# muyangyi/SimSeg

Measured on AMD Instinct MI355X. Metric: image-text pairs/sec (train) + seg images/sec (eval), ViT-B, higher is better.
Workload: dtype fp16

## Files before the change

### include/simseg_hip.h

```cpp
#ifndef SIMSEG_HIP_H
#define SIMSEG_HIP_H
#include <stdint.h>
#ifdef __cplusplus
extern "C" {
#endif

int simseg_version(void);
int simseg_set_half_type(int t);
const char* simseg_last_error(void);

int simseg_gemm(const void* A, const void* B, void* C, int64_t M, int64_t N, int64_t K, int64_t lda, int64_t ldb,
                int64_t ldc, int in_dtype, int out_dtype, int transA, int transB, float alpha, const float* bias,
                const float* rowscale, const float* residual, int64_t ldr, int act, const void* aux, void* aux_out,
                int row_group, int res_mod, int accumulate, int splitk, uint64_t drop_seed, float drop_p, float* colsum,
                void* stream);
int simseg_gemm_aux_blocked_ok(int64_t M, int64_t N, int64_t K);

int simseg_patch_text_sim(const void* x, const void* text, float* out, int64_t M, int64_t C, int64_t K, int dtype, float eps,
                          int normalize, void* stream);

int simseg_set_gemm_variant(int v);
int simseg_gemm_last_variant(void);

int simseg_layernorm_fwd(const float* x, const float* gamma, const float* beta, void* y, int out_dtype, void* y_bf16,
                         float* mean, float* rstd, int64_t rows, int64_t D, float eps, void* stream);
int simseg_layernorm_bwd(const void* dy_bf16, const float* dy_f32, const float* dres, const void* dres_bf16, const float* x,
                         const void* y_bf16, const float* beta, const float* mean,
                         const float* rstd, const float* gamma, float* dx_f32, void* dx_bf16, float* dgamma,
                         float* dbeta, float* dxsum, float* partials, int64_t rows, int64_t D, uint64_t drop_seed, float drop_p,
                         void* stream);
int64_t simseg_layernorm_bwd_workspace_bytes(int64_t rows, int64_t D);

int simseg_colsum_accum(const void* in, int in_dtype, float* out, int64_t rows, int64_t N, int64_t ld, void* stream);

int simseg_vit_im2col(const float* image, void* cols, int out_dtype, int64_t B, int64_t H, int64_t W, void* stream);
int simseg_vit_cls_rows(const float* cls, const float* pos, float* x, int64_t B, int64_t T, int64_t D, void* stream);
int simseg_vit_cls_grad(const float* dx, float* dcls, int64_t B, int64_t T, int64_t D, void* stream);

int simseg_bert_embed_fwd(const int64_t* ids, const float* word, const float* pos, const float* type0, float* out,
                          int64_t B, int64_t L, int64_t D, int64_t vocab, void* stream);
int simseg_bert_embed_bwd(const int64_t* ids, const int64_t* mask, const float* dsum, float* dword, int64_t B, int64_t L,
                          int64_t D, int64_t vocab, void* stream);

int simseg_topk_pool_l2norm_fwd(const void* tok, int dtype, const int64_t* mask, float* emb, int32_t* idx, float* norm,
                                float* scratch, int64_t B, int64_t N, int64_t P, int k, float eps, int normalize, void* stream);
int64_t simseg_topk_pool_workspace_bytes(int64_t B, int64_t P, int k);
int simseg_topk_pool_l2norm_bwd(const float* demb, const float* emb, const float* norm, const int32_t* idx, void* dtok,
                                int dtype, int64_t B, int64_t N, int64_t P, int k, float eps, int normalize, void* stream);

int simseg_set_attention_variant(int v);
int simseg_debug_attn_trace(void* buf);
int simseg_debug_gemm_trace(void* buf);
int simseg_debug_gemm_stagger(int ticks);
int simseg_debug_gemm_wgrad_blocks(int blocks);

// ... 143 lines not shown
```

### simseg_amd/csrc/gemm.hip

```cpp
#include "common.h"

#ifdef SS_GEMM_ABLATE
#define SS_ABL(v) (p.stagger == (v))
#else
#define SS_ABL(v) false
#endif

namespace {

constexpr int BM = 128, BN = 128, NTHREADS = 256;
constexpr int MC_PITCH = 320;
template <int KB> struct Geo {
    static constexpr int KC_PITCH = KB + 16;
    static constexpr int NCH = KB / 16;
    static constexpr int LOADS = 128 * NCH / NTHREADS;
    static constexpr int KROWS = KB / 2;
    static constexpr int TILE_BYTES = (128 * KC_PITCH > KROWS * MC_PITCH) ? 128 * KC_PITCH : KROWS * MC_PITCH;
    static constexpr int KSTEPS = KB / 32;
};

struct GemmParams {
    const void* A; const void* B; void* C;
    int M, N, K;
    long lda, ldb, ldc;
    float alpha;
    const float* bias;
    const float* rowscale;
    const float* residual;
    long ldr;
    int act;
    const void* aux;
    void* aux_out;
    int row_group;
// ... 988 lines not shown
    const int cl = lane & 31, h2 = lane >> 5;
    const float bL = p.bias ? p.bias[c0 + cl] : 0.f, bR = p.bias ? p.bias[c1 + cl] : 0.f;
    float* Cf = reinterpret_cast<float*>(p.C);
    f32x16 rl[2], rr[2];
    auto load_res = [&](int i, f32x16& xl, f32x16& xr) {
        const int row0 = m0 + (i >> 1) * 128 + grp * 64 + (i & 1) * 32;
#pragma unroll
        for (int e = 0; e < 16; ++e) {
            const long ro = (long)(row0 + (e & 3) + 8 * (e >> 2) + 4 * h2) * p.ldr;
            xl[e] = __builtin_nontemporal_load(p.residual + ro + c0 + cl);
            xr[e] = __builtin_nontemporal_load(p.residual + ro + c1 + cl);
        }
    };
    if (p.residual) load_res(0, rl[0], rr[0]);
#pragma unroll
    for (int i = 0; i < 4; ++i) {
        if (p.residual && i < 3) load_res(i + 1, rl[(i + 1) & 1], rr[(i + 1) & 1]);
        const int row0 = m0 + (i >> 1) * 128 + grp * 64 + (i & 1) * 32;
#pragma unroll
        for (int e = 0; e < 16; ++e) {
            const int row = row0 + (e & 3) + 8 * (e >> 2) + 4 * h2;
            float vl = acc[i][0][e] * p.alpha + bL, vr = acc[i][1][e] * p.alpha + bR;
            if (p.drop_thresh) {
                vl = dropout_keep(p.drop_seed, (unsigned long long)row * p.N + c0 + cl, p.drop_thresh) ? vl * p.drop_scale : 0.f;
                vr = dropout_keep(p.drop_seed, (unsigned long long)row * p.N + c1 + cl, p.drop_thresh) ? vr * p.drop_scale : 0.f;
            }
            if (p.residual) { vl += rl[i & 1][e]; vr += rr[i & 1][e]; }
            Cf[(long)row * p.ldc + c0 + cl] = vl;
            Cf[(long)row * p.ldc + c1 + cl] = vr;
        }
    }
}

template <typename TO, bool TA, bool TB, int PP_LEAD = 4, int PRIO = 1, int BIG = 0, int EK = 1>
__global__ __launch_bounds__(512, 2) void gemm_pp_kernel(GemmParams p) {
    extern __shared__ __attribute__((aligned(16))) char lds[];
    const int tid = threadIdx.x, lane = tid & 63, wave = __builtin_amdgcn_readfirstlane(tid >> 6);
    const int grp = wave >> 2, wn = wave & 3;
    const int tiles_n = (p.N + 255) / 256;
    const int tiles = tiles_n * ((p.M + 255) / 256);
    const int q = xcd_remap(blockIdx.x, gridDim.x);
    const int kz = q / tiles, t = q - kz * tiles;
    const int m0 = (t / tiles_n) * 256, n0 = (t % tiles_n) * 256;
    const int nk = p.K / 64;
    const int kt0 = kz * p.ksplit;
    const int ntile = min(nk, kt0 + p.ksplit) - kt0;
    const int stot = 4 * ntile;
    const char* Ab = static_cast<const char*>(p.A) + (TA ? (long)kt0 * 64 * p.lda * 2 : (long)kt0 * 128);
    const char* Bb = static_cast<const char*>(p.B) + (TB ? (long)kt0 * 64 * p.ldb * 2 : (long)kt0 * 128);
    const long astep = TA ? 64 * p.lda * 2 : 128, bstep = TB ? 64 * p.ldb * 2 : 128;
    long dA = 0, dB = 0;
    bool pf_ok = false;
    if (BIG && p.pf_next && p.nsplit == 1) {
        const int nb8 = (int)gridDim.x >> 3, rr8 = (int)gridDim.x & 7, xx = (int)blockIdx.x & 7, jj = (int)blockIdx.x >> 3;
        if (jj + 32 < nb8 + (xx < rr8 ? 1 : 0)) {
            const int tn_ = t + 32;
            const int m1 = (tn_ / tiles_n) * 256, n1 = (tn_ % tiles_n) * 256;
            if (m0 + 256 <= p.M && n0 + 256 <= p.N && m1 + 256 <= p.M && n1 + 256 <= p.N) {
                pf_ok = true;
                dA = TA ? (long)(m1 - m0) * 2 : (long)(m1 - m0) * p.lda * 2;
                dB = TB ? (long)(n1 - n0) * 2 : (long)(n1 - n0) * p.ldb * 2;
            }
        }
    }
    unsigned offA[2][2], offB[2][2];
#pragma unroll
    for (int h = 0; h < 2; ++h)
#pragma unroll
        for (int i = 0; i < 2; ++i) {
            offA[h][i] = pp_src_off<TA>(wave * 2 + i, lane, m0 + h * 128, p.M, p.lda);
            offB[h][i] = pp_src_off<TB>(wave * 2 + i, lane, n0 + h * 128, p.N, p.ldb);
            asm volatile("" : "+v"(offA[h][i]), "+v"(offB[h][i]));
        }
    const unsigned lds0 = (unsigned)(unsigned long)(__attribute__((address_space(3))) char*)lds;
    PPFrag<TA, 2> fra;
// ... 112 lines not shown
#undef PP_CLUSTER
    if (!pf_ok) wait_vm<0>();
    if (grp == 0) __builtin_amdgcn_s_barrier();
    if (p.dbg_trace) tr2 = wall_clock64();

    const bool atomic = p.nsplit > 1;
    const bool vec_ok = epilogue_vec_ok(p, sizeof(TO));
    float* wlds = reinterpret_cast<float*>(lds) + wave * EP_WAVE_FLOATS;
    float cs[8] = {0.f, 0.f, 0.f, 0.f, 0.f, 0.f, 0.f, 0.f};
    const int c0 = n0 + wn * 32, c1 = c0 + 128;
    if constexpr (sizeof(TO) == 2) {
        const bool fastep = !atomic && vec_ok && !p.residual && !p.rowscale && p.row_group == 0 && !p.drop_thresh && !p.dbg_skip_epilogue &&
                            (p.act == 0 || p.act == 1 || (p.act == 3 && (!p.aux_blocked || (EK == 2 && p.aux_blocked == 1) || (EK == 4 && p.aux_blocked == 2))) ||
                             (((EK == 1 && !p.aux_blocked) || (EK == 3 && p.aux_blocked == 1) || (EK == 5 && p.aux_blocked == 2)) && p.act == 4 && p.aux)) && (p.act == 4 || !p.colsum) &&
                            m0 + 256 <= p.M && n0 + 256 <= p.N;
        if (fastep) {
            pp_epilogue_bf16<EK>(p, acc, reinterpret_cast<char*>(wlds), m0, c0, c1, grp, lane);
            if (pf_ok) wait_vm<16>();
            if (p.dbg_trace && tid == 0) {
                const unsigned long long tr3 = wall_clock64();
                asm volatile("s_waitcnt vmcnt(0)" ::: "memory");
                unsigned long long* d = p.dbg_trace + (long)blockIdx.x * 5;
                d[0] = tr0; d[1] = tr1; d[2] = tr2; d[3] = wall_clock64(); d[4] = tr3;
            }
            return;
        }
    }
    if constexpr (sizeof(TO) == 4) {
        const bool direct = !atomic && !p.rowscale && !p.aux && p.act == 0 && p.row_group == 0 && !p.colsum && !p.accumulate &&
                            !p.dbg_skip_epilogue && m0 + 256 <= p.M && n0 + 256 <= p.N;
        if (direct) {
            pp_epilogue_f32_direct(p, acc, m0, c0, c1, grp, lane);
            if (pf_ok) wait_vm<63>();
            if (p.dbg_trace && tid == 0) {
                const unsigned long long tr3 = wall_clock64();
                asm volatile("s_waitcnt vmcnt(0)" ::: "memory");
                unsigned long long* d = p.dbg_trace + (long)blockIdx.x * 5;
                d[0] = tr0; d[1] = tr1; d[2] = tr2; d[3] = wall_clock64(); d[4] = tr3;
            }
            return;
        }
    }
#pragma unroll 1
    for (int i = 0; i < 4; ++i) {
        f32x16 l = acc[0][0], r = acc[0][1];
#pragma unroll
        for (int ii = 1; ii < 4; ++ii)
            if (ii == i) { l = acc[ii][0]; r = acc[ii][1]; }
        if (p.dbg_trace && tid == 0) p.dbg_trace[(long)gridDim.x * 5 + (long)blockIdx.x * 4 + i] = wall_clock64();
        epilogue_block<TO>(p, l, r, wlds, m0 + (i >> 1) * 128 + grp * 64 + (i & 1) * 32, c0, c1, lane, atomic, vec_ok, cs);
    }
    flush_colsum(p, cs, c0, c1, lane);
    if (pf_ok) wait_vm<0>();
    if (p.dbg_trace && tid == 0) {
        const unsigned long long tr3 = wall_clock64();
        asm volatile("s_waitcnt vmcnt(0)" ::: "memory");
        unsigned long long* d = p.dbg_trace + (long)blockIdx.x * 5;
        d[0] = tr0; d[1] = tr1; d[2] = tr2; d[3] = wall_clock64(); d[4] = tr3;
    }
}

template <typename TO, bool TA, bool TB, int LEAD = 4, int PRIO = 1, int BIG = 0, int EK = 1>
int launch_pp(const GemmParams& p, int splitk, hipStream_t stream) {
    constexpr int SMEM = 9 * PP_HALF;
    static bool configured = false;
    auto kern = gemm_pp_kernel<TO, TA, TB, LEAD, PRIO, BIG, EK>;
// ... 485 lines not shown
    return 0;
}
extern "C" int simseg_debug_gemm_trace(void* buf) { g_gemm_debug_trace = static_cast<unsigned long long*>(buf); return 0; }

extern "C" int simseg_set_gemm_variant(int v) {
#ifndef SS_HALF
    simseg_set_gemm_variant_h16(v);
#endif
    g_gemm_debug_skip_epilogue = v >= 100;
    g_gemm_variant = v % 100;
    return 0;
}

namespace {
}

extern "C" int simseg_patch_text_sim(const void* x, const void* text, float* out, int64_t M, int64_t C, int64_t K, int dtype,
                                     float eps, int normalize, void* stream) {
    SS_HALF_FWD(simseg_patch_text_sim, x, text, out, M, C, K, dtype, eps, normalize, stream);
    SS_CHECK(x && text && out, "patch_text_sim: null pointer");
    SS_CHECK(M > 0 && C > 0 && C <= 256 && K > 0 && M < (1ll << 31), "patch_text_sim: need 1 <= C <= 256 (got C=%lld)", (long long)C);
    SS_CHECK(dtype == 0 || dtype == 1, "patch_text_sim: dtype must be 0 (fp32) or 1 (bf16)");
    const int epc = dtype == 0 ? 4 : 8;
    SS_CHECK(K % epc == 0 && ((uintptr_t)x % 16) == 0 && ((uintptr_t)text % 16) == 0, "patch_text_sim: K must be a multiple of %d and the operands 16-byte aligned", epc);
    if (dtype == 0) return dispatch_simmap<float>(x, text, out, (int)M, (int)C, (int)K, eps, normalize, (hipStream_t)stream);
    return dispatch_simmap<bf16_t>(x, text, out, (int)M, (int)C, (int)K, eps, normalize, (hipStream_t)stream);
}

extern "C" int simseg_gemm_aux_blocked_ok(int64_t M, int64_t N, int64_t K) {
    if (M <= 0 || N <= 0 || K <= 0 || M % 256 || N % 256 || K % 64 || K < 768) return 0;
    return (M / 256) * (N / 256) >= 96;
}

extern "C" int simseg_gemm(const void* A, const void* B, void* C, int64_t M, int64_t N, int64_t K, int64_t lda,
                           int64_t ldb, int64_t ldc, int in_dtype, int out_dtype, int transA, int transB, float alpha,
                           const float* bias, const float* rowscale, const float* residual, int64_t ldr, int act,
                           const void* aux, void* aux_out, int row_group, int res_mod, int accumulate, int splitk,
                           uint64_t drop_seed, float drop_p, float* colsum, void* stream) {
    SS_HALF_FWD(simseg_gemm, A, B, C, M, N, K, lda, ldb, ldc, in_dtype, out_dtype, transA, transB, alpha, bias, rowscale, residual, ldr, act, aux, aux_out, row_group, res_mod, accumulate, splitk, drop_seed, drop_p, colsum, stream);
    SS_CHECK(A && B && C, "simseg_gemm: null operand");
    SS_CHECK(M > 0 && N > 0 && K > 0 && M < (1ll << 31) && N < (1ll << 31) && K < (1ll << 31), "simseg_gemm: bad shape %lld x %lld x %lld",
             (long long)M, (long long)N, (long long)K);
    const int epc = in_dtype == 0 ? 4 : 8;
    SS_CHECK(in_dtype == 0 || in_dtype == 1, "simseg_gemm: in_dtype must be 0 (fp32) or 1 (bf16)");
    SS_CHECK(out_dtype == 0 || out_dtype == 1, "simseg_gemm: out_dtype must be 0 (fp32) or 1 (bf16)");
    SS_CHECK(in_dtype == 1 || out_dtype == 0, "simseg_gemm: fp32 operands produce fp32 output");
    SS_CHECK(in_dtype == 1 || (!transA && !transB), "simseg_gemm: transposed operands need bf16");
    SS_CHECK(!(transA && !transB), "simseg_gemm: (transA, !transB) is not on the path");
    const bool aligned = ((uintptr_t)A % 16) == 0 && ((uintptr_t)B % 16) == 0 && lda % epc == 0 && ldb % epc == 0 &&
                         (transA ? M : K) % epc == 0 && (transB ? N : K) % epc == 0;
    SS_CHECK(aligned || in_dtype == 0, "simseg_gemm: bf16 operands need 16-byte aligned pointers and contiguous extents / leading dimensions that are multiples of 8");
    SS_CHECK(((uintptr_t)A % 4) == 0 && ((uintptr_t)B % 4) == 0, "simseg_gemm: misaligned operand");
    SS_CHECK(splitk <= 1 || (out_dtype == 0 && act == 0 && !bias && !residual && drop_p == 0.f && !colsum),
             "simseg_gemm: split-K needs a plain fp32 accumulate epilogue");
    SS_CHECK(drop_p >= 0.f && drop_p < 1.f, "simseg_gemm: dropout p out of range");
    SS_CHECK(act >= 0 && act <= 8, "simseg_gemm: act must be 0..8");
    const int blocked = act >= 7 ? 2 : (act >= 5 ? 1 : 0);
    if (blocked) {
        const bool fwd = act == 5 || act == 7;
        SS_CHECK(simseg_gemm_aux_blocked_ok(M, N, K) && in_dtype == 1 && out_dtype == 1 && !transA && !rowscale && !residual && row_group == 0 &&
                 drop_p == 0.f && splitk <= 1 && ldc == N && (fwd ? aux_out != nullptr : aux != nullptr) &&
                 ((uintptr_t)(fwd ? aux_out : aux) % 16) == 0 && ((uintptr_t)C % 16) == 0 && (!bias || ((uintptr_t)bias % 16) == 0),
                 "simseg_gemm: act %d needs a full-tile 16-bit problem on the ping-pong kernel (simseg_gemm_aux_blocked_ok) with a plain epilogue", act);
        act = fwd ? 3 : 4;
    }
    SS_CHECK((act != 2 && act != 4) || aux, "simseg_gemm: act=2/4 needs aux");
// ... 29 lines not shown
```

### simseg_amd/csrc/half_names.h

```cpp
#pragma once
#ifdef SS_HALF
#define simseg_gemm_last_variant simseg_gemm_last_variant_h16
#define simseg_debug_gemm_stagger simseg_debug_gemm_stagger_h16
#define simseg_debug_gemm_wgrad_blocks simseg_debug_gemm_wgrad_blocks_h16
#define simseg_debug_gemm_trace simseg_debug_gemm_trace_h16
#define simseg_set_gemm_variant simseg_set_gemm_variant_h16
#define simseg_patch_text_sim simseg_patch_text_sim_h16
#define simseg_gemm_aux_blocked_ok simseg_gemm_aux_blocked_ok_h16
#define simseg_gemm simseg_gemm_h16
#define simseg_colsum_accum simseg_colsum_accum_h16
#define simseg_debug_attn_trace simseg_debug_attn_trace_h16
#define simseg_set_attention_variant simseg_set_attention_variant_h16
#define simseg_attention_fwd simseg_attention_fwd_h16
#define simseg_attention_fwd_qscaled simseg_attention_fwd_qscaled_h16
#define simseg_attention_fwd_x3 simseg_attention_fwd_x3_h16
#define simseg_debug_attention_timeline simseg_debug_attention_timeline_h16
#define simseg_attention_bwd_workspace_bytes simseg_attention_bwd_workspace_bytes_h16
#define simseg_attention_bwd simseg_attention_bwd_h16
#define simseg_attention_fwd_rows simseg_attention_fwd_rows_h16
#define simseg_attention_bwd_rows simseg_attention_bwd_rows_h16
#define simseg_attention_fwd_planes simseg_attention_fwd_planes_h16
#define simseg_attention_bwd_planes simseg_attention_bwd_planes_h16
#define simseg_layernorm_fwd simseg_layernorm_fwd_h16
#define simseg_layernorm_bwd simseg_layernorm_bwd_h16
#define simseg_layernorm_bwd_workspace_bytes simseg_layernorm_bwd_workspace_bytes_h16
#define simseg_vit_im2col simseg_vit_im2col_h16
#define simseg_vit_cls_rows simseg_vit_cls_rows_h16
#define simseg_vit_cls_grad simseg_vit_cls_grad_h16
#define simseg_bert_embed_fwd simseg_bert_embed_fwd_h16
#define simseg_bert_embed_bwd simseg_bert_embed_bwd_h16
#define simseg_topk_pool_workspace_bytes simseg_topk_pool_workspace_bytes_h16
#define simseg_topk_pool_l2norm_fwd simseg_topk_pool_l2norm_fwd_h16
#define simseg_topk_pool_l2norm_bwd simseg_topk_pool_l2norm_bwd_h16
#define simseg_segment_mean_l2norm simseg_segment_mean_l2norm_h16
#define simseg_row_rnorm simseg_row_rnorm_h16
#define simseg_cast simseg_cast_h16
#define simseg_split_bf16x3 simseg_split_bf16x3_h16
#define simseg_transpose_f32 simseg_transpose_f32_h16
#define simseg_gather_rows simseg_gather_rows_h16
#define simseg_dropout_apply simseg_dropout_apply_h16
#define simseg_nce_rows simseg_nce_rows_h16
#define simseg_nce_pair simseg_nce_pair_h16
#define simseg_transpose_multi simseg_transpose_multi_h16
#define simseg_scale_rows simseg_scale_rows_h16
#define simseg_scale_by_scalar simseg_scale_by_scalar_h16
#define simseg_retrieval_rank simseg_retrieval_rank_h16
#define simseg_retrieval_rank_cols simseg_retrieval_rank_cols_h16
#define simseg_recall_counts simseg_recall_counts_h16
#define simseg_adamw_multi_step simseg_adamw_multi_step_h16
#define simseg_adamw_multi_step_clip simseg_adamw_multi_step_clip_h16
#define simseg_adamw_multi_step_amp simseg_adamw_multi_step_amp_h16
#define simseg_adamw_multi_step_amp_clip simseg_adamw_multi_step_amp_clip_h16
#define simseg_grads_nonfinite simseg_grads_nonfinite_h16
#define simseg_grads_norm_partials simseg_grads_norm_partials_h16
#define simseg_grads_norm_finish simseg_grads_norm_finish_h16
#define simseg_adamw_step simseg_adamw_step_h16
#else
extern "C" {
int simseg_gemm_last_variant_h16(void);
int simseg_debug_gemm_stagger_h16(int ticks);
int simseg_debug_gemm_wgrad_blocks_h16(int blocks);
int simseg_debug_gemm_trace_h16(void* buf);
int simseg_set_gemm_variant_h16(int v);
int simseg_patch_text_sim_h16(const void* x, const void* text, float* out, int64_t M, int64_t C, int64_t K, int dtype, float eps, int normalize, void* stream);
int simseg_gemm_aux_blocked_ok_h16(int64_t M, int64_t N, int64_t K);
int simseg_gemm_h16(const void* A, const void* B, void* C, int64_t M, int64_t N, int64_t K, int64_t lda, int64_t ldb, int64_t ldc, int in_dtype, int out_dtype, int transA, int transB, float alpha, const float* bias, const float* rowscale, const float* residual, int64_t ldr, int act, const void* aux, void* aux_out, int row_group, int res_mod, int accumulate, int splitk, uint64_t drop_seed, float drop_p, float* colsum, void* stream);
int simseg_colsum_accum_h16(const void* in, int in_dtype, float* out, int64_t rows, int64_t N, int64_t ld, void* stream);
int simseg_debug_attn_trace_h16(void* buf);
int simseg_set_attention_variant_h16(int v);
int simseg_attention_fwd_h16(const void* qkv, const int64_t* key_mask, void* out, float* lse, int dtype, int64_t B, int64_t T, int64_t H, float scale, uint64_t drop_seed, float drop_p, int skip_padded_rows, void* stream);
int simseg_attention_fwd_qscaled_h16(const void* qkv, void* out, float* lse, int64_t B, int64_t T, int64_t H, void* stream);
int simseg_attention_fwd_x3_h16(const void* qkv3, int64_t plane_elems, float* out, int64_t B, int64_t T, int64_t H, float scale, void* stream);
int simseg_debug_attention_timeline_h16(const void* qkv, void* out, float* lse, void* dbg, int64_t B, int64_t T, int64_t H, void* stream);
int64_t simseg_attention_bwd_workspace_bytes_h16(int64_t B, int64_t T, int64_t H);
int simseg_attention_bwd_h16(const void* qkv, const int64_t* key_mask, const void* out, const void* dout, const float* lse, float* workspace, void* dqkv, float* dqkv_colsum, int dtype, int64_t B, int64_t T, int64_t H, float scale, uint64_t drop_seed, float drop_p, int skip_padded_rows, void* stream);
int simseg_attention_fwd_rows_h16(const void* qkv, const int32_t* row_start, void* out, float* lse, int64_t B, int64_t T, int64_t H, float scale, uint64_t drop_seed, float drop_p, void* stream);
int simseg_attention_bwd_rows_h16(const void* qkv, const int32_t* row_start, const void* out, const void* dout, const float* lse, float* workspace, void* dqkv, float* dqkv_colsum, int64_t B, int64_t T, int64_t H, float scale, uint64_t drop_seed, float drop_p, void* stream);
int simseg_attention_fwd_planes_h16(const void* qkv, int64_t plane_rows, const int32_t* row_start, void* out, float* lse, int64_t B, int64_t T, int64_t H, float scale, uint64_t drop_seed, float drop_p, void* stream);
int simseg_attention_bwd_planes_h16(const void* qkv, int64_t plane_rows, const int32_t* row_start, const void* out, const void* dout, const float* lse, float* workspace, void* dqkv, float* dqkv_colsum, int64_t B, int64_t T, int64_t H, float scale, uint64_t drop_seed, float drop_p, void* stream);
int simseg_layernorm_fwd_h16(const float* x, const float* gamma, const float* beta, void* y, int out_dtype, void* y_bf16, float* mean, float* rstd, int64_t rows, int64_t D, float eps, void* stream);
int simseg_layernorm_bwd_h16(const void* dy_bf16, const float* dy_f32, const float* dres, const void* dres_bf16, const float* x, const void* y_bf16, const float* beta, const float* mean, const float* rstd, const float* gamma, float* dx_f32, void* dx_bf16, float* dgamma, float* dbeta, float* dxsum, float* partials, int64_t rows, int64_t D, uint64_t drop_seed, float drop_p, void* stream);
int64_t simseg_layernorm_bwd_workspace_bytes_h16(int64_t rows, int64_t D);
int simseg_vit_im2col_h16(const float* image, void* cols, int out_dtype, int64_t B, int64_t H, int64_t W, void* stream);
int simseg_vit_cls_rows_h16(const float* cls, const float* pos, float* x, int64_t B, int64_t T, int64_t D, void* stream);
int simseg_vit_cls_grad_h16(const float* dx, float* dcls, int64_t B, int64_t T, int64_t D, void* stream);
int simseg_bert_embed_fwd_h16(const int64_t* ids, const float* word, const float* pos, const float* type0, float* out, int64_t B, int64_t L, int64_t D, int64_t vocab, void* stream);
int simseg_bert_embed_bwd_h16(const int64_t* ids, const int64_t* mask, const float* dsum, float* dword, int64_t B, int64_t L, int64_t D, int64_t vocab, void* stream);
int64_t simseg_topk_pool_workspace_bytes_h16(int64_t B, int64_t P, int k);
int simseg_topk_pool_l2norm_fwd_h16(const void* tok, int dtype, const int64_t* mask, float* emb, int32_t* idx, float* norm, float* scratch, int64_t B, int64_t N, int64_t P, int k, float eps, int normalize, void* stream);
int simseg_topk_pool_l2norm_bwd_h16(const float* demb, const float* emb, const float* norm, const int32_t* idx, void* dtok, int dtype, int64_t B, int64_t N, int64_t P, int k, float eps, int normalize, void* stream);
int simseg_segment_mean_l2norm_h16(const float* x, float* out, int64_t S, int64_t P, int64_t D, void* stream);
int simseg_row_rnorm_h16(const void* x, int dtype, float* rnorm, int64_t rows, int64_t D, float eps, void* stream);
int simseg_cast_h16(const void* in, void* out, int64_t n, int to_bf16, void* stream);
int simseg_split_bf16x3_h16(const float* in, void* out, int64_t rows, int64_t K, int64_t ld_in, int b_pattern, void* stream);
int simseg_transpose_f32_h16(const float* in, float* out, int64_t R, int64_t C, void* stream);
int simseg_gather_rows_h16(const void* src, const int32_t* idx, void* dst, int64_t n, int64_t row_bytes, void* stream);
int simseg_dropout_apply_h16(void* g, int dtype, int64_t n, uint64_t seed, float p, void* stream);
int simseg_nce_rows_h16(float* sims, const float* temperature, const float* ignore_mask, float* row_loss, float* row_correct, float* row_tdot, float* out3, int64_t N1, int64_t N2, int64_t target0, float smoothing, int write_grad, void* stream);
// ... 18 lines not shown
```

### simseg_amd/ops.py

```python
import os
import threading

import torch

from .lib import call, ptr, require_gpu, stream, raw

F32, BF16 = 0, 1
_DT = {torch.float32: F32, torch.bfloat16: BF16, torch.float16: BF16}
HALF_TYPES = (torch.bfloat16, torch.float16)


def dt(t):
    try:
        return _DT[t.dtype]
    except KeyError:
        raise TypeError(f"simseg_amd supports fp32, bf16 and fp16 tensors, got {t.dtype}")


def _c(t):
    if t is not None and not t.is_contiguous():
        raise ValueError("simseg_amd ops need contiguous tensors")
    return t


_VARIANT = {"gemm": int(os.environ.get("SIMSEG_GEMM_VARIANT", "0")), "attention": int(os.environ.get("SIMSEG_ATTN_VARIANT", "0"))}
_PUSHED = threading.local()


def _push_variant(kind):
    want = _VARIANT[kind]
    if getattr(_PUSHED, kind, 0) != want:
        call(f"simseg_set_{kind}_variant", want)
# ... 25 lines not shown
    M, K = (a.shape[1], a.shape[0]) if trans_a else (a.shape[0], a.shape[1])
    N = b.shape[1] if trans_b else b.shape[0]
    kb = b.shape[0] if trans_b else b.shape[1]
    if kb != K:
        raise ValueError(f"gemm: inner dims differ ({K} vs {kb})")
    if act in (7, 8):
        t8 = aux_out if act == 7 else aux
        if t8 is None or t8.dtype != torch.uint8 or t8.numel() < a.shape[0] * (b.shape[1] if trans_b else b.shape[0]):
            raise TypeError("gemm: act 7 / 8 take the derivative image as a uint8 tensor of M x N bytes")
    if a.dtype != b.dtype or (aux is not None and act != 8 and aux.dtype not in (a.dtype, torch.float32)):
        raise TypeError(f"gemm: operands of different types ({a.dtype}, {b.dtype}{'' if aux is None else ', aux ' + str(aux.dtype)}): bf16 and fp16 do not mix in one call")
    if out is None:
        rows = out_rows if out_rows is not None else M
        out = torch.empty(rows, N, device=a.device, dtype=out_dtype or a.dtype)
    _c(out)
    ldr = residual.shape[-1] if residual is not None else 0
    _push_variant("gemm")
    if PROFILE is not None:
        e0, e1 = torch.cuda.Event(enable_timing=True), torch.cuda.Event(enable_timing=True)
        e0.record()
    call("simseg_gemm", ptr(a), ptr(b), ptr(out), M, N, K, a.shape[1], b.shape[1], out.shape[-1], dt(a), dt(out),
         int(trans_a), int(trans_b), float(alpha), ptr(_c(bias)), ptr(_c(rowscale)), ptr(_c(residual)), ldr, int(act),
         ptr(_c(aux)), ptr(_c(aux_out)), int(row_group), int(res_mod), int(accumulate), int(splitk), int(drop_seed),
         float(drop_p), ptr(colsum), stream())
    if PROFILE is not None:
        e1.record()
        kind = ("f32" if a.dtype == torch.float32 else "bf16") + "_" + ("t" if trans_a else "n") + ("n" if trans_b else "t")
        kind += "_o32" if out.dtype == torch.float32 else "_o16"
        kind += {1: "", 2: "_L", 3: "_P", 4: "_S", 5: "_R", 8: "_X", 9: "_Y", 10: "_Q"}[raw("simseg_gemm_last_variant")]
        PROFILE.append((kind, 2.0 * M * N * K, e0, e1))
    return out


_BLK_OK = {}


def gemm_aux_blocked_ok(M, N, K):
    key = (int(M), int(N), int(K))
    r = _BLK_OK.get(key)
    if r is None:
        r = _BLK_OK[key] = os.environ.get("SIMSEG_AMD_BLOCKED_AUX", "1") != "0" and bool(raw("simseg_gemm_aux_blocked_ok", *key))
    return r


def layernorm_fwd(x, gamma, beta, eps, out_dtype=torch.float32, want_bf16_copy=False, save_stats=False):
    require_gpu(x)
    D = x.shape[-1]
    rows = x.numel() // D
    y = torch.empty(x.shape, device=x.device, dtype=out_dtype)
    y16 = torch.empty(x.shape, device=x.device, dtype=want_bf16_copy if isinstance(want_bf16_copy, torch.dtype) else torch.bfloat16) if want_bf16_copy else None
    mean = torch.empty(rows, device=x.device, dtype=torch.float32) if save_stats else None
    rstd = torch.empty(rows, device=x.device, dtype=torch.float32) if save_stats else None
    call("simseg_layernorm_fwd", ptr(_c(x)), ptr(gamma), ptr(beta), ptr(y), dt(y), ptr(y16), ptr(mean), ptr(rstd), rows, D,
         float(eps), stream())
    return y, y16, mean, rstd


def layernorm_bwd(x, mean, rstd, gamma, dgamma, dbeta, dy16=None, dy32=None, dres=None, want_f32=True, want_bf16=True,
                  dxsum=None, drop_seed=0, drop_p=0.0, dres16=None, y16=None, beta=None):
    require_gpu(x)
    D = x.shape[-1]
    rows = x.numel() // D
    dx32 = torch.empty(x.shape, device=x.device, dtype=torch.float32) if want_f32 else None
    h16 = dy16.dtype if dy16 is not None else (want_bf16 if isinstance(want_bf16, torch.dtype) else torch.bfloat16)
    dx16 = torch.empty(x.shape, device=x.device, dtype=h16) if want_bf16 else None
    partials = torch.empty(raw("simseg_layernorm_bwd_workspace_bytes", rows, D) // 4, device=x.device, dtype=torch.float32)
# ... 706 lines not shown
```

### simseg_amd/towers.py

```python
import contextlib
import os
import weakref

import torch
from torch.autograd import Function

from . import ops

BF16, F32 = torch.bfloat16, torch.float32


_W16 = {}


def weights_rewritten(param, w16):
    _W16[id(param)] = (weakref.ref(param), param._version, param.data_ptr(), w16)
    _W3.pop(id(param), None)
    for key in _WQS_OF.pop(id(param), ()):
        _WQS.pop(key, None)


def invalidate_weight_cache():
    _W16.clear()
    _CAT.clear()
# ... 200 lines not shown
            return fn(ctx, *grads)
        finally:
            _wg_join()
    return wrapped


def _wgrad(dy, x, out=None):
    if _WG_ON and dy.is_cuda:
        cur = torch.cuda.current_stream()
        side = _wg_side(cur)
        if out is None:
            out = torch.zeros(dy.shape[1], x.shape[1], device=dy.device, dtype=F32)
        side.wait_stream(cur)
        with torch.cuda.stream(side):
            _wgrad_now(dy, x, out)
        pend = getattr(_WG_PENDING, "streams", None)
        if pend is None:
            pend = _WG_PENDING.streams = []
        if side not in pend:
            pend.append(side)
        return out
    return _wgrad_now(dy, x, out)


def _wgrad_now(dy, x, out=None):
    out_f, in_f = dy.shape[1], x.shape[1]
    dw = torch.zeros(out_f, in_f, device=dy.device, dtype=F32) if out is None else out
    sk = _splitk(out_f, in_f, dy.shape[0])
    if dy.dtype == F32:
        ops.gemm(ops.transpose_f32(dy), ops.transpose_f32(x), out=dw, accumulate=True, splitk=sk)
    else:
        ops.gemm(dy, x, trans_a=True, trans_b=True, out=dw, accumulate=True, splitk=sk)
    return dw


def _dgrad(d, w_, **kw):
    if d.dtype == F32:
        return ops.gemm(d, ops.transpose_f32(w_), **kw)
    return ops.gemm(d, w_, trans_b=True, **kw)


_FUSED_QKV_BIAS = os.environ.get("SIMSEG_AMD_FUSED_QKV_BIAS", "1") != "0"


def _zeros_like_bias(out, n, device):
    return torch.zeros(n, device=device, dtype=F32) if out is None else out


def _bgrad(dy, out=None):
    db = torch.zeros(dy.shape[1], device=dy.device, dtype=F32) if out is None else out
    ops.colsum_accum(dy, db)
    return db


def _act_grad(t32, adt):
    return t32 if adt == F32 else ops.cast(t32, adt)


def _ln_bwd(adt, x, mean, rstd, w, dg, db, dy, dres=None, dy32=None, dxsum=None, drop=(0.0, 0), dres16=None, want32=True, y16=None, beta=None):
    if adt != F32:
        if not (_XHAT_Y and y16 is not None and beta is not None):
            y16 = beta = None
        return ops.layernorm_bwd(x, mean, rstd, w, dg, db, dy16=dy, dy32=dy32, dres=dres, dres16=dres16, dxsum=dxsum, drop_seed=drop[1], drop_p=drop[0],
                                 want_bf16=adt, want_f32=want32, y16=y16, beta=beta)
    if dy32 is not None:
        raise ValueError("exact mode: fold the second gradient into `dy` with the producing GEMM's residual epilogue")
# ... 159 lines not shown
        g8 = blk and _GELU8
        pre = torch.empty(B * T, 4 * D, device=x.device, dtype=torch.uint8 if g8 else adt) if save else None
        act = ops.gemm(ln2, f1w_, bias=f1b.detach(), act=((7 if g8 else 5) if blk else 3) if save else 1, aux_out=pre)
        y = ops.gemm(act, f2w_, bias=f2b.detach(), residual=x1, out_dtype=F32)
        ctx.adt, ctx.heads, ctx.dims, ctx.blk = adt, heads, (B, T, D), (2 if g8 else 1) if blk else 0
        ctx.lazy = bool(lazy_ok) and adt != F32 and _RES16
        ctx.wparams = (f2w, f1w, pw, qw)
        if save:
            ctx.save_for_backward(x, mean1, rstd1, ln1, qkv, att, lse, x1, mean2, rstd2, ln2, pre, act, qw_, pw_, f1w_, f2w_,
                                  n1w.detach(), n2w.detach(), n1b.detach(), n2b.detach())
        return y.view(B, T, D)

    @staticmethod
    @_joins_wgrad
    def backward(ctx, dy):
        x, mean1, rstd1, ln1, qkv, att, lse, x1, mean2, rstd2, ln2, pre, act, qw_, pw_, f1w_, f2w_, n1w, n2w, n1b, n2b = ctx.saved_tensors
        B, T, D = ctx.dims
        adt = ctx.adt
        need = ctx.needs_input_grad
        dy = dy.contiguous()
        sh = _take_shadow(dy, adt) if adt != F32 else None
        _need_shadow(dy, sh)
        res16 = sh is not None and adt != F32 and _RES16
        dy = dy.view(-1, D)
        if sh is not None:
            dy16, df2b = sh[0].view(-1, D), sh[1]
        else:
            dy16 = _act_grad(dy, adt)
            df2b = _bgrad(dy16) if need[14] else None
        tg = [_grad_target(w) if nd else None for w, nd in zip(ctx.wparams, (need[13], need[11], need[7], need[5]))]
        (df1b, df2w_z, df1w_z, dn2w, dn2b, dpb, dpw_z, dqw_z, dqb_z, dn1w, dn1b, dsum) = _zeros_or(
            dy.device, (None, tg[0], tg[1], None, None, None, tg[2], tg[3], None, None, None, None),
            (4 * D,), (D, 4 * D), (4 * D, D), (D,), (D,), (D,), (D, D), (3 * D, D), (3 * D,), (D,), (D,), (D,))
        dpre = _dgrad(dy16, f2w_, act=(4, 6, 8)[ctx.blk], aux=pre, colsum=df1b)
        df2w = _wgrad(dy16, act, df2w_z) if need[13] else None
        dln2 = _dgrad(dpre, f1w_)
        df1w = _wgrad(dpre, ln2, df1w_z) if need[11] else None
        r16 = adt != F32 and _RES16
        dx1_32, dx1_16 = _ln_bwd(adt, x1, mean2, rstd2, n2w, dn2w, dn2b, dln2, dres=None if res16 else dy, dres16=dy16 if res16 else None, dxsum=dpb,
                                 want32=not r16, y16=ln2, beta=n2b)
        datt = _dgrad(dx1_16, pw_)
        dpw = _wgrad(dx1_16, att.view(-1, D), dpw_z) if need[7] else None
        dqb = _zeros_like_bias(dqb_z, 3 * D, qkv.device) if need[6] else None
        dqkv = ops.attention_bwd(qkv.view(B, T, 3 * D), att, datt.view(B, T, D), lse, ctx.heads, None, scale=64 ** -0.5,
                                 colsum=dqb if _FUSED_QKV_BIAS else None).view(-1, 3 * D)
        if dqb is not None and not _FUSED_QKV_BIAS:
            ops.colsum_accum(dqkv, dqb)
        dln1 = _dgrad(dqkv, qw_)
        dqw = _wgrad(dqkv, ln1.view(-1, D), dqw_z) if need[5] else None
        dx, dx16 = _ln_bwd(adt, x.view(-1, D), mean1, rstd1, n1w, dn1w, dn1b, dln1, dres=None if r16 else dx1_32, dres16=dx1_16 if r16 else None,
                           dxsum=dsum, want32=not ctx.lazy, y16=ln1, beta=n1b)
        if dx is None:
            dx = _lazy32((B, T, D), x.device, dx16, dsum)
        else:
            dx = dx.view(B, T, D)
            if adt != F32:
                _put_shadow(dx, dx16, dsum)
        return (dx, None, None, dn1w, dn1b, dqw, dqb, dpw, dpb, dn2w, dn2b, df1w, df1b, df2w, df2b, None)


def vit_forward(m, image, adt):
    x = ViTEmbedFn.apply(image, m.patch_embed.proj.weight, m.patch_embed.proj.bias, m.cls_token, m.pos_embed, adt)
    for blk in m.blocks:
        x = ViTBlockFn.apply(x, m.num_heads, adt, blk.norm1.weight, blk.norm1.bias, blk.attn.qkv.weight, blk.attn.qkv.bias,
                             blk.attn.proj.weight, blk.attn.proj.bias, blk.norm2.weight, blk.norm2.bias,
                             blk.mlp.fc1.weight, blk.mlp.fc1.bias, blk.mlp.fc2.weight, blk.mlp.fc2.bias, True)
    return LayerNormFn.apply(x, m.norm.weight, m.norm.bias, 1e-6, adt, True)


class BertEmbedFn(Function):

    @staticmethod
    def forward(ctx, ids, mask, word, pos, typ, lnw, lnb, drop_p, seed):
        B, L = ids.shape
        if L > pos.shape[0]:
            raise ValueError(f"sequence length {L} exceeds max_position_embeddings {pos.shape[0]}")
        s = ops.bert_embed_fwd(ids.contiguous(), word.detach(), pos.detach(), typ.detach()[0].contiguous())
        y, _, mean, rstd = ops.layernorm_fwd(s, lnw.detach(), lnb.detach(), 1e-12, save_stats=True)
        if drop_p > 0:
            ops.dropout_apply_(y, seed, drop_p)
        ctx.drop = (drop_p, seed)
        ctx.shapes = (word.shape, pos.shape, typ.shape)
        ctx.wparams = (word,)
        ctx.save_for_backward(ids, mask, s, mean, rstd, lnw.detach())
# ... 164 lines not shown
        aa = a32 if adt == F32 else a16
        blk = save and adt != F32 and ops.gemm_aux_blocked_ok(aa.shape[0], iw.shape[0], D)
        g8 = blk and _GELU8
        pre = torch.empty(x.shape[0] if packed else B * L, iw.shape[0], device=x.device, dtype=torch.uint8 if g8 else adt) if save else None
        act = _fwd_gemm(aa, iw, adt, save, bias=ib.detach(), act=((7 if g8 else 5) if blk else 3) if save else 1, aux_out=pre)
        s2 = _fwd_gemm(act, o2w, adt, save, bias=o2b.detach(), residual=a32, out_dtype=F32, drop_seed=seed + 2, drop_p=drop_p)
        y, y16, mean_o, rstd_o = ops.layernorm_fwd(s2, low.detach(), lob.detach(), 1e-12, want_bf16_copy=(adt if (adt != F32 and packed) else False), save_stats=save)
        if y16 is not None:
            y._simseg_fwd16 = (y16, y._version)
        ctx.adt, ctx.heads, ctx.dims, ctx.drop, ctx.packed, ctx.rows, ctx.nv, ctx.blk = adt, heads, (B, L, D), (drop_p, seed), packed, rows, nv, (2 if g8 else 1) if blk else 0
        ctx.wparams = (o2w, iw, ow)
        if save:
            ctx.save_for_backward(xa, mask, qkv, att, lse, s1, mean_a, rstd_a, aa, pre, act, s2, mean_o, rstd_o, wqkv, ow_, iw_, o2w_,
                                  law.detach(), low.detach(), attd if (packed and not rows) else None, idx, inv, cu if rows else None)
        return y if packed else y.view(B, L, D)

    @staticmethod
    @_joins_wgrad
    def backward(ctx, dy):
        (xa, mask, qkv, att, lse, s1, mean_a, rstd_a, aa, pre, act, s2, mean_o, rstd_o, wqkv, ow_, iw_, o2w_, law, low, attd, idx, inv, cu) = ctx.saved_tensors
        B, L, D = ctx.dims
        packed = ctx.packed
        adt = ctx.adt
        p, seed = ctx.drop
        need = ctx.needs_input_grad
        dy = dy.contiguous().view(-1, D)
        I = pre.shape[1]
        tg = [_grad_target(w) if nd else None for w, nd in zip(ctx.wparams, (need[18], need[16], need[12]))]
        (dlow, dlob, do2b, dib, do2w_z, diw_z, dlaw, dlab, dob, dow_z, dwqkv_z, dbqkv_z) = _zeros_or(
            dy.device, (None, None, None, None, tg[0], tg[1], None, None, None, tg[2], None, None),
            (D,), (D,), (D,), (I,), (D, I), (I, D), (D,), (D,), (D,), (D, D), (3 * D, D), (3 * D,))
        ds2_32, d2 = _ln_bwd(adt, s2, mean_o, rstd_o, low, dlow, dlob, None if adt != F32 else dy, dy32=dy if adt != F32 else None,
                             dxsum=do2b, drop=(p, seed + 2))
        dpre = _dgrad(d2, o2w_, act=(4, 6, 8)[ctx.blk], aux=pre, colsum=dib)
        do2w = _wgrad(d2, act, do2w_z) if need[18] else None
        da = _dgrad(dpre, iw_) if adt != F32 else _dgrad(dpre, iw_, residual=ds2_32)
        diw = _wgrad(dpre, aa, diw_z) if need[16] else None
        ds1_32, d1 = _ln_bwd(adt, s1, mean_a, rstd_a, law, dlaw, dlab, da, dy32=ds2_32 if adt != F32 else None, dxsum=dob,
                             drop=(p, seed + 1))
        datt = _dgrad(d1, ow_)
        dow = _wgrad(d1, att.view(-1, D), dow_z) if need[12] else None
        dbqkv = _zeros_like_bias(dbqkv_z, 3 * D, qkv.device) if (need[7] or need[9] or need[11]) else None
        if ctx.rows:
            dqkv = ops.attention_bwd_rows(qkv, att, datt.contiguous(), lse, ctx.heads, cu, L, scale=64 ** -0.5, drop_seed=seed, drop_p=p,
                                          colsum=dbqkv if _FUSED_QKV_BIAS else None, n_real=ctx.nv)
        else:
            if packed:
                datt = ops.gather_rows(datt, inv)
            dqkv = ops.attention_bwd(qkv.view(B, L, 3 * D), (attd if packed else att).view(B, L, D), datt.view(B, L, D), lse, ctx.heads, mask,
                                     scale=64 ** -0.5, drop_seed=seed, drop_p=p, skip_padded_rows=packed and _SKIP_PAD,
                                     colsum=dbqkv if _FUSED_QKV_BIAS else None, zero_skipped=False).view(-1, 3 * D)
            if packed:
                dqkv = ops.gather_rows(dqkv, idx)
        if dbqkv is not None and not _FUSED_QKV_BIAS:
            ops.colsum_accum(dqkv, dbqkv)
        dx = _dgrad(dqkv, wqkv, residual=ds1_32, out_dtype=F32)
        dwqkv = _wgrad(dqkv, xa, dwqkv_z) if (need[6] or need[8] or need[10]) else None
        dws = [dwqkv[i * D:(i + 1) * D] if dwqkv is not None else None for i in range(3)]
        dbs = [dbqkv[i * D:(i + 1) * D] if dbqkv is not None else None for i in range(3)]
        return (dx if packed else dx.view(B, L, D), None, None, None, None, None, dws[0], dbs[0], dws[1], dbs[1], dws[2], dbs[2], dow, dob,
                dlaw, dlab, diw, dib, do2w, do2b, dlow, dlob, None, None, None, None)


_PACK_TEXT = [False, None]
_SKIP_PAD = os.environ.get("SIMSEG_AMD_SKIP_PAD_ROWS", "1") != "0"


@contextlib.contextmanager
def packed_text(lengths=None):
    prev = list(_PACK_TEXT)
    _PACK_TEXT[0] = os.environ.get("SIMSEG_AMD_PACKED_TEXT", "1") != "0"
    _PACK_TEXT[1] = lengths
    try:
        yield
    finally:
        _PACK_TEXT[:] = prev


def bert_forward(m, input_ids, attention_mask, adt, training=False, seed=0):
    p_h = m.hidden_dropout_prob if training else 0.0
    p_a = m.attention_probs_dropout_prob if training else 0.0
    if p_h != p_a:
        raise NotImplementedError("hidden and attention dropout probabilities are expected to be equal (HF default 0.1)")
    e = m.embeddings
    mask = attention_mask.contiguous().long()
    x = BertEmbedFn.apply(input_ids, mask, e.word_embeddings.weight, e.position_embeddings.weight, e.token_type_embeddings.weight,
                          e.LayerNorm.weight, e.LayerNorm.bias, p_h, seed)
    B, L, D = x.shape
    idx = inv = cu = None
    nv = 0
# ... 73 lines not shown
```

Baseline: 5799.

## Batch per-block weight-gradient GEMMs into one grouped split-K launch

Weight-gradient GEMMs of a transformer block are no longer launched one by one. They are deferred and issued together in a single grouped kernel that maps blocks to problems through prefix offsets, with the split-K factor chosen by a simple cost model over all tiles. An atomic-add direct epilogue is added for the split-K fp32 accumulation. The aim is fewer launches and better CU fill for small wgrad GEMMs, at the cost of atomic contention, a longer live range for the deferred activations, and a fallback path when shapes are not 256-aligned.

```diff
diff --git a/include/simseg_hip.h b/include/simseg_hip.h
--- a/include/simseg_hip.h
+++ b/include/simseg_hip.h
@@ -21,6 +21,9 @@
 
 int simseg_set_gemm_variant(int v);
 int simseg_gemm_last_variant(void);
+
+int simseg_gemm_wgrad_group(const int64_t* problems, int n, int64_t rows, int slices, void* stream);
+int simseg_wgrad_group_last(void);
 
 int simseg_layernorm_fwd(const float* x, const float* gamma, const float* beta, void* y, int out_dtype, void* y_bf16,
                          float* mean, float* rstd, int64_t rows, int64_t D, float eps, void* stream);
diff --git a/simseg_amd/csrc/gemm.hip b/simseg_amd/csrc/gemm.hip
--- a/simseg_amd/csrc/gemm.hip
+++ b/simseg_amd/csrc/gemm.hip
@@ -1,4 +1,5 @@
 #include "common.h"
+#include <type_traits>
 
 #ifdef SS_GEMM_ABLATE
 #define SS_ABL(v) (p.stagger == (v))
@@ -1053,15 +1054,70 @@
     }
 }
 
-template <typename TO, bool TA, bool TB, int PP_LEAD = 4, int PRIO = 1, int BIG = 0, int EK = 1>
-__global__ __launch_bounds__(512, 2) void gemm_pp_kernel(GemmParams p) {
+__device__ __forceinline__ void pp_epilogue_atomic_direct(const GemmParams& p, const f32x16 (&acc)[4][2], int m0, int c0, int c1, int grp, int lane) {
+    const int cl = lane & 31, h2 = lane >> 5;
+    float* Cf = reinterpret_cast<float*>(p.C);
+#pragma unroll
+    for (int i = 0; i < 4; ++i) {
+        float* Cr = Cf + (long)(m0 + (i >> 1) * 128 + grp * 64 + (i & 1) * 32 + 4 * h2) * p.ldc + cl;
+#pragma unroll
+        for (int e = 0; e < 16; ++e) {
+            float* Ce = Cr + (long)((e & 3) + 8 * (e >> 2)) * p.ldc;
+            atomicAdd(Ce + c0, acc[i][0][e] * p.alpha);
+            atomicAdd(Ce + c1, acc[i][1][e] * p.alpha);
+        }
+    }
+}
+
+constexpr int WG_MAX = 8;
+struct WgradProblem {
+    const void* dy; const void* x; float* dw;
+    long ld_dy, ld_x, ld_dw;
+    int out, in;
+};
+struct WgradGroupParams {
+    WgradProblem prob[WG_MAX];
+    int first[WG_MAX + 1];
+    int n, rows, ksplit, nsplit;
+    unsigned long long* dbg_trace;
+};
+
+__device__ __forceinline__ const GemmParams& pp_params(const GemmParams& arg, const GemmParams&) { return arg; }
+__device__ __forceinline__ const GemmParams& pp_params(const WgradGroupParams&, const GemmParams& own) { return own; }
+
+template <typename TO, bool TA, bool TB, int PP_LEAD = 4, int PRIO = 1, int BIG = 0, int EK = 1, bool GROUPED = false, bool ATOMIC_DIRECT = false>
+__global__ __launch_bounds__(512, 2) void gemm_pp_kernel(typename std::conditional<GROUPED, WgradGroupParams, GemmParams>::type arg) {
     extern __shared__ __attribute__((aligned(16))) char lds[];
+    GemmParams own;
+    int gkz = 0, gt = 0;
+    if constexpr (GROUPED) {
+        const int gq = xcd_remap(blockIdx.x, gridDim.x);
+        if (gq >= arg.first[arg.n]) return;
+        int i = 0;
+#pragma unroll
+        for (int j = 1; j < WG_MAX; ++j)
+            if (j < arg.n && gq >= arg.first[j]) i = j;
+        const WgradProblem& w = arg.prob[i];
+        own = GemmParams{};
+        own.A = w.dy; own.B = w.x; own.C = w.dw;
+        own.M = w.out; own.N = w.in; own.K = arg.rows;
+        own.lda = w.ld_dy; own.ldb = w.ld_x; own.ldc = w.ld_dw;
+        own.alpha = 1.0f;
+        own.accumulate = 1;
+        own.ksplit = arg.ksplit; own.nsplit = arg.nsplit;
+        own.dbg_trace = arg.dbg_trace;
+        const int gtiles = (w.out >> 8) * (w.in >> 8);
+        const int r = gq - arg.first[i];
+        gkz = r / gtiles;
+        gt = r - gkz * gtiles;
+    }
+    const GemmParams& p = pp_params(arg, own);
     const int tid = threadIdx.x, lane = tid & 63, wave = __builtin_amdgcn_readfirstlane(tid >> 6);
     const int grp = wave >> 2, wn = wave & 3;
     const int tiles_n = (p.N + 255) / 256;
     const int tiles = tiles_n * ((p.M + 255) / 256);
     const int q = xcd_remap(blockIdx.x, gridDim.x);
-    const int kz = q / tiles, t = q - kz * tiles;
+    const int kz = GROUPED ? gkz : q / tiles, t = GROUPED ? gt : q - kz * tiles;
     const int m0 = (t / tiles_n) * 256, n0 = (t % tiles_n) * 256;
     const int nk = p.K / 64;
     const int kt0 = kz * p.ksplit;
@@ -1240,6 +1296,18 @@
         if (direct) {
             pp_epilogue_f32_direct(p, acc, m0, c0, c1, grp, lane);
             if (pf_ok) wait_vm<63>();
+            if (p.dbg_trace && tid == 0) {
+                const unsigned long long tr3 = wall_clock64();
+                asm volatile("s_waitcnt vmcnt(0)" ::: "memory");
+                unsigned long long* d = p.dbg_trace + (long)blockIdx.x * 5;
+                d[0] = tr0; d[1] = tr1; d[2] = tr2; d[3] = wall_clock64(); d[4] = tr3;
+            }
+            return;
+        }
+    }
+    if constexpr (ATOMIC_DIRECT && sizeof(TO) == 4) {
+        if (atomic && !p.dbg_skip_epilogue && m0 + 256 <= p.M && n0 + 256 <= p.N) {
+            pp_epilogue_atomic_direct(p, acc, m0, c0, c1, grp, lane);
             if (p.dbg_trace && tid == 0) {
                 const unsigned long long tr3 = wall_clock64();
                 asm volatile("s_waitcnt vmcnt(0)" ::: "memory");
@@ -1791,6 +1859,59 @@
     return (M / 256) * (N / 256) >= 96;
 }
 
+static thread_local int g_wgrad_group_last = 0;
+extern "C" int simseg_wgrad_group_last(void) {
+    SS_HALF_FWD(simseg_wgrad_group_last); return g_wgrad_group_last; }
+
+extern "C" int simseg_gemm_wgrad_group(const int64_t* problems, int n, int64_t rows, int slices, void* stream) {
+    SS_HALF_FWD(simseg_gemm_wgrad_group, problems, n, rows, slices, stream);
+    g_wgrad_group_last = 0;
+    SS_CHECK(problems && n >= 1 && n <= WG_MAX, "simseg_gemm_wgrad_group: 1..%d problems", WG_MAX);
+    SS_CHECK(rows > 0 && rows < (1ll << 31) && slices >= 1, "simseg_gemm_wgrad_group: bad rows %lld / slices %d", (long long)rows, slices);
+    if (rows % 64 != 0) return 0;
+    const int nk = (int)(rows / 64);
+    if (nk / slices < 16) return 0;
+    WgradGroupParams g;
+    memset(&g, 0, sizeof(g));
+    g.ksplit = (nk + slices - 1) / slices;
+    g.nsplit = (nk + g.ksplit - 1) / g.ksplit;
+    long blocks = 0;
+    for (int i = 0; i < n; ++i) {
+        const int64_t* d = problems + 8 * i;
+        WgradProblem& w = g.prob[i];
+        SS_CHECK(d[0] && d[1] && d[2], "simseg_gemm_wgrad_group: null operand in problem %d", i);
+        const int64_t out = d[3], in = d[4];
+        if (out <= 0 || in <= 0 || out % 256 || in % 256 || out >= (1ll << 31) || in >= (1ll << 31)) return 0;
+        if (d[5] < out || d[6] < in || d[7] < in || d[5] % 8 || d[6] % 8 || d[7] % 4) return 0;
+        if ((uintptr_t)d[0] % 16 || (uintptr_t)d[1] % 16 || (uintptr_t)d[2] % 16) return 0;
+        if (64 * d[5] * 2 >= (1ll << 31) || 64 * d[6] * 2 >= (1ll << 31)) return 0;
+        w.dy = (const void*)(uintptr_t)d[0]; w.x = (const void*)(uintptr_t)d[1]; w.dw = (float*)(uintptr_t)d[2];
+        w.out = (int)out; w.in = (int)in; w.ld_dy = d[5]; w.ld_x = d[6]; w.ld_dw = d[7];
+        g.first[i] = (int)blocks;
+        blocks += (out / 256) * (in / 256) * g.nsplit;
+        if (blocks >= (1l << 24)) return 0;
+    }
+    for (int i = n; i <= WG_MAX; ++i) g.first[i] = (int)blocks;
+    g.n = n; g.rows = (int)rows;
+    g.dbg_trace = g_gemm_debug_trace;
+    static const bool direct = !(getenv("SIMSEG_GEMM_WGRAD_DIRECT") && atoi(getenv("SIMSEG_GEMM_WGRAD_DIRECT")) == 0);
+    constexpr int SMEM = 9 * PP_HALF;
+    static bool configured = false;
+    if (!configured) {
+        hipError_t e = hipFuncSetAttribute(reinterpret_cast<const void*>(&gemm_pp_kernel<float, true, true, 4, 1, 1, 1, true, false>), hipFuncAttributeMaxDynamicSharedMemorySize, SMEM);
+        if (e == hipSuccess) e = hipFuncSetAttribute(reinterpret_cast<const void*>(&gemm_pp_kernel<float, true, true, 4, 1, 1, 1, true, true>), hipFuncAttributeMaxDynamicSharedMemorySize, SMEM);
+        if (e != hipSuccess) return simseg_set_error("simseg_gemm_wgrad_group: cannot reserve %d bytes of LDS: %s", SMEM, hipGetErrorString(e));
+        configured = true;
+    }
+    hipStream_t s = (hipStream_t)stream;
+    if (direct) hipLaunchKernelGGL((gemm_pp_kernel<float, true, true, 4, 1, 1, 1, true, true>), dim3((unsigned)blocks, 1, 1), dim3(512), SMEM, s, g);
+    else hipLaunchKernelGGL((gemm_pp_kernel<float, true, true, 4, 1, 1, 1, true, false>), dim3((unsigned)blocks, 1, 1), dim3(512), SMEM, s, g);
+    SS_LAUNCH_CHECK("simseg_gemm_wgrad_group");
+    g_gemm_last_variant = 3;
+    g_wgrad_group_last = n;
+    return 0;
+}
+
 extern "C" int simseg_gemm(const void* A, const void* B, void* C, int64_t M, int64_t N, int64_t K, int64_t lda,
                            int64_t ldb, int64_t ldc, int in_dtype, int out_dtype, int transA, int transB, float alpha,
                            const float* bias, const float* rowscale, const float* residual, int64_t ldr, int act,
diff --git a/simseg_amd/csrc/half_names.h b/simseg_amd/csrc/half_names.h
--- a/simseg_amd/csrc/half_names.h
+++ b/simseg_amd/csrc/half_names.h
@@ -7,6 +7,8 @@
 #define simseg_set_gemm_variant simseg_set_gemm_variant_h16
 #define simseg_patch_text_sim simseg_patch_text_sim_h16
 #define simseg_gemm_aux_blocked_ok simseg_gemm_aux_blocked_ok_h16
+#define simseg_wgrad_group_last simseg_wgrad_group_last_h16
+#define simseg_gemm_wgrad_group simseg_gemm_wgrad_group_h16
 #define simseg_gemm simseg_gemm_h16
 #define simseg_colsum_accum simseg_colsum_accum_h16
 #define simseg_debug_attn_trace simseg_debug_attn_trace_h16
@@ -64,6 +66,8 @@
 int simseg_set_gemm_variant_h16(int v);
 int simseg_patch_text_sim_h16(const void* x, const void* text, float* out, int64_t M, int64_t C, int64_t K, int dtype, float eps, int normalize, void* stream);
 int simseg_gemm_aux_blocked_ok_h16(int64_t M, int64_t N, int64_t K);
+int simseg_wgrad_group_last_h16(void);
+int simseg_gemm_wgrad_group_h16(const int64_t* problems, int n, int64_t rows, int slices, void* stream);
 int simseg_gemm_h16(const void* A, const void* B, void* C, int64_t M, int64_t N, int64_t K, int64_t lda, int64_t ldb, int64_t ldc, int in_dtype, int out_dtype, int transA, int transB, float alpha, const float* bias, const float* rowscale, const float* residual, int64_t ldr, int act, const void* aux, void* aux_out, int row_group, int res_mod, int accumulate, int splitk, uint64_t drop_seed, float drop_p, float* colsum, void* stream);
 int simseg_colsum_accum_h16(const void* in, int in_dtype, float* out, int64_t rows, int64_t N, int64_t ld, void* stream);
 int simseg_debug_attn_trace_h16(void* buf);
diff --git a/simseg_amd/ops.py b/simseg_amd/ops.py
--- a/simseg_amd/ops.py
+++ b/simseg_amd/ops.py
@@ -1,3 +1,4 @@
+import ctypes
 import os
 import threading
 
@@ -89,6 +90,74 @@
     return out
 
 
+def gemm_last_variant():
+    return raw("simseg_gemm_last_variant")
+
+
+WGRAD_EPILOGUE_KTILES = 8
+
+
+def wgrad_group_plan(tiles, nk, cus=256):
+    total = int(sum(tiles))
+    nk = int(nk)
+    best, best_cost = 1, None
+    for sk in range(1, max(1, nk // 16) + 1):
+        cost = -(-total * sk // cus) * (-(-nk // sk) + WGRAD_EPILOGUE_KTILES)
+        if best_cost is None or cost < best_cost:
+            best, best_cost = sk, cost
+    return best
+
+
+_WG_LAST = threading.local()
+
+
+def wgrad_group_last():
+    return getattr(_WG_LAST, "n", 0)
+
+
+def wgrad_group(problems, slices=None):
+    problems = list(problems)
+    if not problems:
+        return
+    rows = problems[0][0].shape[0]
+    ok = 1 <= len(problems) <= 8
+    for dy, x, out in problems:
+        require_gpu(dy, x, out)
+        _c(dy); _c(x); _c(out)
+        if dy.dim() != 2 or x.dim() != 2 or dy.shape[0] != x.shape[0] or tuple(out.shape) != (dy.shape[1], x.shape[1]) or out.dtype != torch.float32:
+            raise ValueError("wgrad_group: need dy [rows, out], x [rows, in] and an fp32 dW [out, in]")
+        if dy.dtype != x.dtype:
+            raise TypeError(f"wgrad_group: operands of different types ({dy.dtype}, {x.dtype})")
+        ok = ok and dy.shape[0] == rows and dy.dtype in HALF_TYPES and dy.dtype == problems[0][0].dtype
+    nk = rows // 64
+    if slices is None:
+        slices = wgrad_group_plan([(dy.shape[1] // 256) * (x.shape[1] // 256) for dy, x, _ in problems], nk)
+    _push_variant("gemm")
+    if PROFILE is not None:
+        e0, e1 = torch.cuda.Event(enable_timing=True), torch.cuda.Event(enable_timing=True)
+        e0.record()
+    grouped = 0
+    if ok:
+        desc = []
+        for dy, x, out in problems:
+            desc += [ptr(dy), ptr(x), ptr(out), dy.shape[1], x.shape[1], dy.shape[1], x.shape[1], x.shape[1]]
+        call("simseg_gemm_wgrad_group", (ctypes.c_int64 * len(desc))(*desc), len(problems), rows, int(slices), stream())
+        grouped = raw("simseg_wgrad_group_last")
+    _WG_LAST.n = grouped
+    if not grouped:
+        for dy, x, out in problems:
+            t128 = -(-dy.shape[1] // 128) * -(-x.shape[1] // 128)
+            sk = max(1, min(-(-dy.shape[0] // 64), -(-1024 // t128), 64))
+            if dy.dtype == torch.float32:
+                gemm(transpose_f32(dy), transpose_f32(x), out=out, accumulate=True, splitk=sk)
+            else:
+                gemm(dy, x, trans_a=True, trans_b=True, out=out, accumulate=True, splitk=sk)
+        return
+    if PROFILE is not None:
+        e1.record()
+        PROFILE.append(("bf16_tn_o32_P", sum(2.0 * dy.shape[1] * x.shape[1] * rows for dy, x, _ in problems), e0, e1))
+
+
 _BLK_OK = {}
 
 
diff --git a/simseg_amd/towers.py b/simseg_amd/towers.py
--- a/simseg_amd/towers.py
+++ b/simseg_amd/towers.py
@@ -256,6 +256,20 @@
     else:
         ops.gemm(dy, x, trans_a=True, trans_b=True, out=dw, accumulate=True, splitk=sk)
     return dw
+
+
+_WG_GROUP = os.environ.get("SIMSEG_AMD_WGRAD_GROUP", "1") != "0"
+WGRAD_GROUPS = [0]
+
+
+def _wgrad_grouped(adt, needs):
+    return _WG_GROUP and not _WG_ON and adt != F32 and all(needs)
+
+
+def _wgrad_flush(group):
+    ops.wgrad_group(group)
+    if ops.wgrad_group_last():
+        WGRAD_GROUPS[0] += 1
 
 
 def _dgrad(d, w_, **kw):
@@ -481,24 +495,28 @@
         (df1b, df2w_z, df1w_z, dn2w, dn2b, dpb, dpw_z, dqw_z, dqb_z, dn1w, dn1b, dsum) = _zeros_or(
             dy.device, (None, tg[0], tg[1], None, None, None, tg[2], tg[3], None, None, None, None),
             (4 * D,), (D, 4 * D), (4 * D, D), (D,), (D,), (D,), (D, D), (3 * D, D), (3 * D,), (D,), (D,), (D,))
+        group = [] if _wgrad_grouped(adt, (need[13], need[11], need[7], need[5])) else None
+        wg = _wgrad if group is None else (lambda d, x_, z: group.append((d, x_, z)) or z)
         dpre = _dgrad(dy16, f2w_, act=(4, 6, 8)[ctx.blk], aux=pre, colsum=df1b)
-        df2w = _wgrad(dy16, act, df2w_z) if need[13] else None
+        df2w = wg(dy16, act, df2w_z) if need[13] else None
         dln2 = _dgrad(dpre, f1w_)
-        df1w = _wgrad(dpre, ln2, df1w_z) if need[11] else None
+        df1w = wg(dpre, ln2, df1w_z) if need[11] else None
         r16 = adt != F32 and _RES16
         dx1_32, dx1_16 = _ln_bwd(adt, x1, mean2, rstd2, n2w, dn2w, dn2b, dln2, dres=None if res16 else dy, dres16=dy16 if res16 else None, dxsum=dpb,
                                  want32=not r16, y16=ln2, beta=n2b)
         datt = _dgrad(dx1_16, pw_)
-        dpw = _wgrad(dx1_16, att.view(-1, D), dpw_z) if need[7] else None
+        dpw = wg(dx1_16, att.view(-1, D), dpw_z) if need[7] else None
         dqb = _zeros_like_bias(dqb_z, 3 * D, qkv.device) if need[6] else None
         dqkv = ops.attention_bwd(qkv.view(B, T, 3 * D), att, datt.view(B, T, D), lse, ctx.heads, None, scale=64 ** -0.5,
                                  colsum=dqb if _FUSED_QKV_BIAS else None).view(-1, 3 * D)
         if dqb is not None and not _FUSED_QKV_BIAS:
             ops.colsum_accum(dqkv, dqb)
         dln1 = _dgrad(dqkv, qw_)
-        dqw = _wgrad(dqkv, ln1.view(-1, D), dqw_z) if need[5] else None
+        dqw = wg(dqkv, ln1.view(-1, D), dqw_z) if need[5] else None
         dx, dx16 = _ln_bwd(adt, x.view(-1, D), mean1, rstd1, n1w, dn1w, dn1b, dln1, dres=None if r16 else dx1_32, dres16=dx1_16 if r16 else None,
                            dxsum=dsum, want32=not ctx.lazy, y16=ln1, beta=n1b)
+        if group:
+            _wgrad_flush(group)
         if dx is None:
             dx = _lazy32((B, T, D), x.device, dx16, dsum)
         else:
@@ -729,14 +747,16 @@
             (D,), (D,), (D,), (I,), (D, I), (I, D), (D,), (D,), (D,), (D, D), (3 * D, D), (3 * D,))
         ds2_32, d2 = _ln_bwd(adt, s2, mean_o, rstd_o, low, dlow, dlob, None if adt != F32 else dy, dy32=dy if adt != F32 else None,
                              dxsum=do2b, drop=(p, seed + 2))
+        group = [] if _wgrad_grouped(adt, (need[18], need[16], need[12], need[6] or need[8] or need[10])) else None
+        wg = _wgrad if group is None else (lambda d, x_, z: group.append((d, x_, z)) or z)
         dpre = _dgrad(d2, o2w_, act=(4, 6, 8)[ctx.blk], aux=pre, colsum=dib)
-        do2w = _wgrad(d2, act, do2w_z) if need[18] else None
+        do2w = wg(d2, act, do2w_z) if need[18] else None
         da = _dgrad(dpre, iw_) if adt != F32 else _dgrad(dpre, iw_, residual=ds2_32)
-        diw = _wgrad(dpre, aa, diw_z) if need[16] else None
+        diw = wg(dpre, aa, diw_z) if need[16] else None
         ds1_32, d1 = _ln_bwd(adt, s1, mean_a, rstd_a, law, dlaw, dlab, da, dy32=ds2_32 if adt != F32 else None, dxsum=dob,
                              drop=(p, seed + 1))
         datt = _dgrad(d1, ow_)
-        dow = _wgrad(d1, att.view(-1, D), dow_z) if need[12] else None
+        dow = wg(d1, att.view(-1, D), dow_z) if need[12] else None
         dbqkv = _zeros_like_bias(dbqkv_z, 3 * D, qkv.device) if (need[7] or need[9] or need[11]) else None
         if ctx.rows:
             dqkv = ops.attention_bwd_rows(qkv, att, datt.contiguous(), lse, ctx.heads, cu, L, scale=64 ** -0.5, drop_seed=seed, drop_p=p,
@@ -752,7 +772,9 @@
         if dbqkv is not None and not _FUSED_QKV_BIAS:
             ops.colsum_accum(dqkv, dbqkv)
         dx = _dgrad(dqkv, wqkv, residual=ds1_32, out_dtype=F32)
-        dwqkv = _wgrad(dqkv, xa, dwqkv_z) if (need[6] or need[8] or need[10]) else None
+        dwqkv = wg(dqkv, xa, dwqkv_z) if (need[6] or need[8] or need[10]) else None
+        if group:
+            _wgrad_flush(group)
         dws = [dwqkv[i * D:(i + 1) * D] if dwqkv is not None else None for i in range(3)]
         dbs = [dbqkv[i * D:(i + 1) * D] if dbqkv is not None else None for i in range(3)]
         return (dx if packed else dx.view(B, L, D), None, None, None, None, None, dws[0], dbs[0], dws[1], dbs[1], dws[2], dbs[2], dow, dob,
```

Result: faster. 5910, median of 6 (+1.9%).
